# happyxtt/CNNs_SLFP_quantization

Measured on AMD Instinct MI355X. Metric: images/sec at batch 256, MobileNetV1 SLFP<3,4> ImageNet-224; % HBM roofline, higher is better.
Workload: dtype f32 (1x1 contraction: fp16 MFMA operands, f32 accumulate); 1 GPU; mobilenetv1_imagenet224: all 27 Conv2d_Q layers, SLFP<3,4> Qbits=8, NHWC, batch 256 per GPU as 2 concurrent image groups of 128 on 2 HIP streams, inputs resident in HBM; batch_per_gpu=256, global_batch=256, parallelism=batch-sharded x1, one-time RCCL broadcast of the u8 weight codes, pointwise_mfma=pw_mfma_f16x1

## Files before the change

cnns_slfp_quantization_amd/_lib.py:

```python
import ctypes
import os

_HERE = os.path.dirname(os.path.abspath(__file__))
LIB_PATH = os.path.join(_HERE, "libslfp_hip.so")

OK, ERR_BAD_ARG, ERR_SHAPE, ERR_UNSUPPORTED, ERR_ALIGNMENT, ERR_HIP = 0, -1, -2, -3, -4, -5
FMT_ACT8, FMT_W8, FMT_SFP7, FMT_EXT = 0, 1, 2, 4
LAYOUT_NCHW, LAYOUT_NHWC = 0, 1
MFMA_DEFAULT, MFMA_F16X1, MFMA_F16X3 = 0, 1, 3
OPT_SGD, OPT_DSGD, OPT_SSGD = 0, 1, 2

SYMBOLS = (
    "slfp_version", "slfp_last_error", "slfp_device_count",
    "slfp_encode_f32", "slfp_decode_f32", "slfp_quantize_f32", "slfp_quantize_layerout_f32", "slfp_absmax_f32",
    "slfp_conv2d_out_shape", "slfp_conv2d_kernel_name", "slfp_conv2d_wprep_bytes",
    "slfp_conv2d_prepare_weights", "slfp_conv2d_prepare_weights_codes", "slfp_conv2d_workspace_bytes", "slfp_conv2d_fwd", "slfp_conv2d_fwd_post",
    "slfp_linear_workspace_bytes", "slfp_linear_fwd", "slfp_linear_prepare_weights", "slfp_linear_fwd_prepared",
    "slfp_nchw_to_nhwc_f32", "slfp_nhwc_to_nchw_f32", "slfp_debug_div_mismatches",
    "slfp_debug_enc_mismatches", "slfp_enc_table_ok", "slfp_dwpw_supported", "slfp_dwpw_fwd",
    "slfp_conv2d_codes_supported", "slfp_conv2d_fwd_codes", "slfp_conv2d_fwd_codes_ws", "slfp_maxpool2d_codes", "slfp_debug_code_mismatches", "slfp_debug_reload_switches",
    "slfp_debug_enc_hl_mismatches", "slfp_sgd_step_f32",
    "slfp_conv2d_bwd_supported", "slfp_conv2d_bwd_kernel_name", "slfp_conv2d_bwd_workspace_bytes", "slfp_conv2d_bwd",
)


class ConvDesc(ctypes.Structure):
    _fields_ = [
        ("n", ctypes.c_int64), ("c_in", ctypes.c_int64), ("h", ctypes.c_int64), ("w", ctypes.c_int64),
        ("c_out", ctypes.c_int64), ("kh", ctypes.c_int64), ("kw", ctypes.c_int64),
        ("stride_h", ctypes.c_int32), ("stride_w", ctypes.c_int32), ("pad_h", ctypes.c_int32),
        ("pad_w", ctypes.c_int32), ("dil_h", ctypes.c_int32), ("dil_w", ctypes.c_int32),
        ("groups", ctypes.c_int32), ("x_layout", ctypes.c_int32), ("y_layout", ctypes.c_int32),
        ("qbits", ctypes.c_int32), ("ka", ctypes.c_float), ("kw_scale", ctypes.c_float),
        ("mfma_passes", ctypes.c_int32), ("reserved", ctypes.c_int32),
    ]


class ConvIo(ctypes.Structure):
    _fields_ = [("x_codes", ctypes.c_int32), ("y_codes", ctypes.c_int32), ("y_ka", ctypes.c_float), ("y_qbits", ctypes.c_int32)]


class SgdHparams(ctypes.Structure):
    _fields_ = [("rule", ctypes.c_int32), ("qbits", ctypes.c_int32), ("lr", ctypes.c_float), ("momentum", ctypes.c_float),
                ("damp_alpha", ctypes.c_float), ("weight_decay", ctypes.c_float), ("nesterov", ctypes.c_int32),
                ("reserved", ctypes.c_int32)]


class SlfpError(RuntimeError):
    def __init__(self, code, text):
        super().__init__(f"libslfp_hip: {text} (status {code})")
        self.code = code


_lib = None


def load():
    global _lib
    if _lib is not None:
        return _lib
    if not os.path.exists(LIB_PATH):
        raise RuntimeError(
            f"{LIB_PATH} is missing: the SLFP HIP extension is not built. "
            "Run `python -m cnns_slfp_quantization_amd.build` (needs hipcc). There is no CPU fallback.")
    import torch
    L = ctypes.CDLL(LIB_PATH)
    vp, sz, ci, cf, i64 = ctypes.c_void_p, ctypes.c_size_t, ctypes.c_int, ctypes.c_float, ctypes.c_int64
    dp = ctypes.POINTER(ConvDesc)
    sigs = {
        "slfp_version": (ci, []),
        "slfp_last_error": (ctypes.c_char_p, []),
        "slfp_device_count": (ci, []),
        "slfp_encode_f32": (ci, [vp, vp, sz, cf, ci, vp]),
        "slfp_decode_f32": (ci, [vp, vp, sz, ci, vp]),
        "slfp_quantize_f32": (ci, [vp, vp, sz, cf, ci, vp]),
        "slfp_quantize_layerout_f32": (ci, [vp, vp, sz, vp]),
        "slfp_absmax_f32": (ci, [vp, sz, vp, vp]),
        "slfp_conv2d_out_shape": (ci, [dp, ctypes.POINTER(i64), ctypes.POINTER(i64)]),
        "slfp_conv2d_kernel_name": (ctypes.c_char_p, [dp]),
        "slfp_conv2d_wprep_bytes": (sz, [dp]),
        "slfp_conv2d_prepare_weights": (ci, [dp, vp, vp, vp, vp]),
        "slfp_conv2d_prepare_weights_codes": (ci, [dp, vp, vp, vp, vp]),
        "slfp_conv2d_workspace_bytes": (sz, [dp]),
        "slfp_conv2d_fwd": (ci, [dp, vp, vp, vp, vp, vp, vp, vp]),
        "slfp_conv2d_fwd_post": (ci, [dp, vp, vp, vp, vp, vp, ci, vp, vp, vp, vp]),
        "slfp_linear_workspace_bytes": (sz, [i64, i64, i64]),
        "slfp_linear_fwd": (ci, [vp, vp, vp, vp, i64, i64, i64, cf, cf, ci, ci, vp, vp]),
        "slfp_linear_prepare_weights": (ci, [vp, vp, i64, i64, cf, ci, ci, vp]),
        "slfp_linear_fwd_prepared": (ci, [vp, vp, vp, vp, i64, i64, i64, cf, cf, ci, ci, vp]),
        "slfp_nchw_to_nhwc_f32": (ci, [vp, vp, i64, i64, i64, i64, vp]),
        "slfp_nhwc_to_nchw_f32": (ci, [vp, vp, i64, i64, i64, i64, vp]),
        "slfp_debug_div_mismatches": (ci, [cf, vp, vp]),
        "slfp_debug_enc_mismatches": (ci, [cf, ci, vp, vp]),
        "slfp_enc_table_ok": (ci, [cf, ci]),
        "slfp_dwpw_supported": (ci, [dp, dp]),
        "slfp_dwpw_fwd": (ci, [dp, dp, vp, vp, vp, vp, ci, vp, vp, vp, vp, ci, vp, vp]),
        "slfp_conv2d_codes_supported": (ci, [dp, ctypes.POINTER(ConvIo), ci, ci]),
        "slfp_conv2d_fwd_codes": (ci, [dp, ctypes.POINTER(ConvIo), vp, vp, vp, vp, vp, ci, vp, vp]),
        "slfp_conv2d_fwd_codes_ws": (ci, [dp, ctypes.POINTER(ConvIo), vp, vp, vp, vp, vp, ci, vp, vp, vp]),
        "slfp_maxpool2d_codes": (ci, [vp, vp, i64, i64, i64, i64, ci, ci, ci, ci, ci, ci, ci, vp]),
        "slfp_debug_code_mismatches": (ci, [cf, ci, vp, vp]),
        "slfp_debug_reload_switches": (None, []),
        "slfp_debug_enc_hl_mismatches": (ci, [cf, ci, vp, vp]),
        "slfp_sgd_step_f32": (ci, [ctypes.POINTER(SgdHparams), sz, vp, vp, vp, vp, vp, vp]),
        "slfp_conv2d_bwd_supported": (ci, [dp]),
        "slfp_conv2d_bwd_kernel_name": (ctypes.c_char_p, [dp]),
        "slfp_conv2d_bwd_workspace_bytes": (sz, [dp, ci, ci]),
        "slfp_conv2d_bwd": (ci, [dp, vp, vp, vp, vp, vp, vp, vp, vp]),
    }
    assert set(sigs) == set(SYMBOLS)
    for name, (res, args) in sigs.items():
        fn = getattr(L, name)
        fn.restype = res
        fn.argtypes = args
    _lib = L
    return L


def last_error():
    return load().slfp_last_error().decode("utf-8", "replace")


def check(rc):
    if rc == OK:
        return
    text = last_error()
    if rc in (ERR_BAD_ARG, ERR_SHAPE):
        raise SlfpError(rc, text)
    raise SlfpError(rc, text)
```

cnns_slfp_quantization_amd/build.py:

```python
import os
import shutil
import subprocess
import sys

HERE = os.path.dirname(os.path.abspath(__file__))
CSRC = os.path.join(HERE, "csrc")
LIB = os.path.join(HERE, "libslfp_hip.so")
SOURCES = ["codec.hip", "enc_table.hip", "conv_dw.hip", "conv_dw2.hip", "conv_dwpw.hip", "conv_dwc.hip", "conv_pw.hip", "conv_pw_codes.hip", "conv_direct.hip", "conv_dense.hip", "conv_stem_mfma.hip", "conv_stem_small.hip", "pool_codes.hip", "optim.hip", "conv_bwd.hip", "conv_abi.hip"]
FLAGS = ["--offload-arch=gfx950", "-O3", "-std=c++17", "-fPIC", "-fno-fast-math", "-ffp-contract=off",
         "-Wall", "-Wno-unused-variable", "-Wno-unused-but-set-variable"]


def _hipcc():
    for cand in (os.environ.get("HIPCC"), shutil.which("hipcc"), "/opt/rocm/bin/hipcc"):
        if cand and os.path.exists(cand):
            return cand
    raise RuntimeError("hipcc not found (set HIPCC or install ROCm)")


def needs_build():
    if not os.path.exists(LIB):
        return True
    t = os.path.getmtime(LIB)
    deps = [os.path.join(CSRC, f) for f in os.listdir(CSRC)] + [os.path.join(HERE, "..", "include", "slfp.h")]
    return any(os.path.getmtime(d) > t for d in deps)


def build(force=False, verbose=False):
    if not force and not needs_build():
        return LIB
    hipcc = _hipcc()
    extra = os.environ.get("SLFP_EXTRA_HIPCC_FLAGS", "").split()
    objdir = os.path.join(HERE, "build")
    os.makedirs(objdir, exist_ok=True)
    procs = []
    for src in SOURCES:
        obj = os.path.join(objdir, src + ".o")
        cmd = [hipcc] + FLAGS + extra + ["-c", os.path.join(CSRC, src), "-o", obj]
        if verbose:
            print(" ".join(cmd), flush=True)
        procs.append((src, obj, subprocess.Popen(cmd, stdout=subprocess.PIPE, stderr=subprocess.STDOUT, text=True)))
    objs = []
    for src, obj, p in procs:
        out, _ = p.communicate()
        if p.returncode != 0:
            raise RuntimeError(f"hipcc failed on {src}:\n{out}")
        if verbose and out.strip():
            print(out)
        objs.append(obj)
    cmd = [hipcc, "--offload-arch=gfx950", "-shared", "-fPIC", "-o", LIB] + objs
    subprocess.check_call(cmd)
    return LIB


if __name__ == "__main__":
    print(build(force="--force" in sys.argv, verbose=True))
```

cnns_slfp_quantization_amd/csrc/codec.hip:

```cpp
#include <cstdarg>
#include <mutex>
#include <map>
#include <set>
#include <utility>
#include <cstdio>
#include "slfp_device.hpp"
#include "slfp_enc.hpp"
#include "slfp_host.hpp"

namespace slfp {

static thread_local char g_err[512] = "";

void set_error(const char* fmt, ...) {
    va_list ap;
    va_start(ap, fmt);
    vsnprintf(g_err, sizeof(g_err), fmt, ap);
    va_end(ap);
}

int fail(int code, const char* fmt, ...) {
    va_list ap;
    va_start(ap, fmt);
    vsnprintf(g_err, sizeof(g_err), fmt, ap);
    va_end(ap);
    return code;
}

int check_launch(const char* what) {
    hipError_t e = hipGetLastError();
    if (e != hipSuccess) return fail(SLFP_ERR_HIP, "%s: %s", what, hipGetErrorString(e));
    return SLFP_OK;
}

const char* last_error_text() { return g_err; }

int raise_lds_limit(const void* fn, size_t lds_bytes) {
    if (lds_bytes <= 48 * 1024) return SLFP_OK;
    static std::mutex mu;
    static std::map<std::pair<int, const void*>, size_t> raised;
    int dev = 0;
    if (hipGetDevice(&dev) != hipSuccess) return check_launch("hipGetDevice");
    std::lock_guard<std::mutex> lock(mu);
    const auto key = std::make_pair(dev, fn);
    const auto it = raised.find(key);
    if (it != raised.end() && it->second >= lds_bytes) return SLFP_OK;
    if (hipFuncSetAttribute(fn, hipFuncAttributeMaxDynamicSharedMemorySize, (int)lds_bytes) != hipSuccess)
        return check_launch("hipFuncSetAttribute(MaxDynamicSharedMemorySize)");
    raised[key] = lds_bytes;
    return SLFP_OK;
}

static Switches read_switches() {
    Switches w;
    w.long_encode = std::getenv("SLFP_LONG_ENCODE") != nullptr;
    w.dw_old = std::getenv("SLFP_DW_OLD") != nullptr;
    w.pw_nostg = std::getenv("SLFP_PW_NOSTG") != nullptr;
    w.pw_notab = std::getenv("SLFP_PW_NOTAB") != nullptr;
    const char* e = std::getenv("SLFP_PW_STG_MAXKS");
    w.pw_stg_maxks = e ? atoi(e) : -1;
    e = std::getenv("SLFP_PW_NT_MIN_MB");
    w.pw_nt_min_mb = e ? atoll(e) : 0;
    e = std::getenv("SLFP_DW_NT_MIN_MB");
    w.dw_nt_min_mb = e ? atoll(e) : 30;
    w.stem_old = std::getenv("SLFP_STEM_OLD") != nullptr;
    w.pwc_slice = std::getenv("SLFP_PWC_NOSLICE") == nullptr;
    w.dense_generic = std::getenv("SLFP_DENSE_GENERIC") != nullptr;
    e = std::getenv("SLFP_DENSE_CFG");
    w.dense_cfg = e ? atoi(e) : 0;
    e = std::getenv("SLFP_DENSE_NWB");
    w.dense_nwb = e ? atoi(e) : 0;
    w.dense_res = std::getenv("SLFP_DENSE_NORES") == nullptr;
    w.dense_encx = std::getenv("SLFP_DENSE_NOENCX") == nullptr;
    w.stem_im2row = std::getenv("SLFP_STEM_IM2ROW") != nullptr;
    e = std::getenv("SLFP_PW_STREAM_MAX_KB");
    w.pw_stream_max_kb = e ? atoi(e) : 30;
    return w;
}
static Switches g_switches = read_switches();
const Switches& switches() { return g_switches; }
void reload_switches() { g_switches = read_switches(); }

int device_cu_count() {
    static std::mutex mu;
    static std::map<int, int> cus;
    int dev = 0;
    if (hipGetDevice(&dev) != hipSuccess) { (void)hipGetLastError(); return 256; }
    std::lock_guard<std::mutex> lock(mu);
    const auto it = cus.find(dev);
    if (it != cus.end()) return it->second;
    int n = 0;
    if (hipDeviceGetAttribute(&n, hipDeviceAttributeMultiprocessorCount, dev) != hipSuccess || n <= 0) { (void)hipGetLastError(); n = 256; }
    cus[dev] = n;
    return n;
}

int resident_blocks_per_cu(const void* fn, int block_threads, size_t dynamic_lds) {
    static std::mutex mu;
    static std::map<std::pair<std::pair<int, const void*>, size_t>, int> cache;
    int dev = 0;
    if (hipGetDevice(&dev) != hipSuccess) { (void)hipGetLastError(); return 1; }
    const auto key = std::make_pair(std::make_pair(dev, fn), dynamic_lds);
    std::lock_guard<std::mutex> lock(mu);
    const auto it = cache.find(key);
    if (it != cache.end()) return it->second;
    int n = 0;
    if (hipOccupancyMaxActiveBlocksPerMultiprocessor(&n, fn, block_threads, dynamic_lds) != hipSuccess || n < 1) { (void)hipGetLastError(); n = 1; }
    cache[key] = n;
    return n;
}

constexpr int kThreads = 256;

template <int FMT, int MODE>
__global__ __launch_bounds__(kThreads) void k_codec(const float* __restrict__ x, void* __restrict__ out,
                                                    size_t n, const ScaleDiv sd, int ext, int vec_ok) {
    __shared__ uint32_t sT[16];
    lut_fill<FMT>(sT);
    __syncthreads();
    const size_t nvec = vec_ok ? n / 4 : 0;
    const size_t stride = (size_t)gridDim.x * kThreads;
    for (size_t i = (size_t)blockIdx.x * kThreads + threadIdx.x; i < nvec; i += stride) {
        const float4 v = reinterpret_cast<const float4*>(x)[i];
        const uint32_t u0 = __float_as_uint(div_const(v.x, sd)), u1 = __float_as_uint(div_const(v.y, sd));
        const uint32_t u2 = __float_as_uint(div_const(v.z, sd)), u3 = __float_as_uint(div_const(v.w, sd));
        if constexpr (MODE == 0) {
            float4 r;
// ... 267 lines not shown
```

cnns_slfp_quantization_amd/csrc/conv_abi.hip:

```cpp
#include <cstring>
#include "slfp_device.hpp"
#include "slfp_codes.hpp"
#include "slfp_host.hpp"

namespace slfp {

static size_t round256(size_t b) { return (b + 255) & ~(size_t)255; }

static int make_plan_core(const slfp_conv2d_desc* d, ConvPlan* plan) {
    if (!d || !plan) return fail(SLFP_ERR_BAD_ARG, "conv2d: null descriptor");
    if (d->n <= 0 || d->c_in <= 0 || d->h <= 0 || d->w <= 0 || d->c_out <= 0 || d->kh <= 0 || d->kw <= 0)
        return fail(SLFP_ERR_SHAPE, "conv2d: non-positive size");
    if (d->stride_h <= 0 || d->stride_w <= 0 || d->dil_h <= 0 || d->dil_w <= 0 || d->pad_h < 0 || d->pad_w < 0)
        return fail(SLFP_ERR_SHAPE, "conv2d: bad stride/dilation/padding");
    if (d->groups <= 0 || d->c_in % d->groups || d->c_out % d->groups)
        return fail(SLFP_ERR_SHAPE, "conv2d: groups=%d does not divide C_in=%lld / C_out=%lld", d->groups,
                    (long long)d->c_in, (long long)d->c_out);
    if (d->qbits != 8 && d->qbits != 7)
        return fail(SLFP_ERR_BAD_ARG, "conv2d: qbits must be 8 (SLFP<3,4>) or 7 (SFP<3,3>), got %d", d->qbits);
    if ((d->x_layout != SLFP_LAYOUT_NCHW && d->x_layout != SLFP_LAYOUT_NHWC) ||
        (d->y_layout != SLFP_LAYOUT_NCHW && d->y_layout != SLFP_LAYOUT_NHWC))
        return fail(SLFP_ERR_BAD_ARG, "conv2d: unknown layout");
    if (!(d->ka > 0.f) || !(d->kw_scale > 0.f)) return fail(SLFP_ERR_BAD_ARG, "conv2d: Ka and Kw must be > 0");
    if (!scale_div_ok(d->ka) || !scale_div_ok(d->kw_scale))
// ... 172 lines not shown
    if (p.family == kPointwise || p.family == kDenseMfma || p.family == kStemMfma || p.family == kStemSmall || p.repad) {
        if (hipMemsetAsync(wprep, 0, p.wprep_bytes, stream) != hipSuccess) return check_launch("hipMemsetAsync(wprep)");
    }
    const int64_t plane = p.family == kStemMfma ? p.n_pad : p.k_pad * p.n_pad;
    const int KS = p.family == kStemMfma ? (int)p.k_pad : (int)(p.k_pad / 32);
    const unsigned grid = (unsigned)ceil_div(total, 256);
    const ScaleDiv sd = make_scale_div(d.kw_scale);
    const int ldo = p.family == kDenseMfma ? (p.passes == 3 ? 1 : 0) : (int)p.cpo;
#define SLFP_PREP(FF, CC) hipLaunchKernelGGL((k_prepare<FF, CC>), dim3(grid), dim3(256), 0, stream, w_oihw, wprep, weight_q_oihw, total, \
                                             (int)d.c_out, Cg, (int)d.kh, (int)d.kw, sd, (int)p.family, KS, plane, ldo)
    if (p.fmt_w == kFmtW8) { if (codes) SLFP_PREP(kFmtW8, true); else SLFP_PREP(kFmtW8, false); }
    else { if (codes) SLFP_PREP(kFmtSfp7, true); else SLFP_PREP(kFmtSfp7, false); }
#undef SLFP_PREP
    return check_launch("slfp weight prepare kernel");
}

static const char* family_name(const ConvPlan& p, const slfp_conv2d_desc& d) {
    if (p.family == kDirect && stem_applicable(d)) return "stem_nhwc";
    if (p.repad) {
        if (p.family == kDw3x3) return "repad+dw3x3_nhwc";
        return p.fmt_act == kFmtSfp7 ? "repad+pw_mfma_f16_exact" : (p.passes == 3 ? "repad+pw_mfma_f16x3" : "repad+pw_mfma_f16x1");
    }
    switch (p.family) {
        case kDw3x3: return "dw3x3_nhwc";
        case kPointwise: return p.fmt_act == kFmtSfp7 ? "pw_mfma_f16_exact" : (p.passes == 3 ? "pw_mfma_f16x3" : "pw_mfma_f16x1");
        case kDenseMfma: return p.fmt_act == kFmtSfp7 ? "dense_mfma_f16_exact" : (p.passes == 3 ? "dense_mfma_f16x3" : "dense_mfma_f16x1");
        case kStemMfma: return p.fmt_act == kFmtSfp7 ? "stem_mfma_f16_exact" : "stem_mfma_f16x1";
        case kStemSmall: return p.fmt_act == kFmtSfp7 ? "stem_small_mfma_f16_exact" : "stem_small_mfma_f16x1";
        default: return "direct_nhwc";
    }
}

}

using namespace slfp;

extern "C" {

int slfp_conv2d_out_shape(const slfp_conv2d_desc* d, int64_t* h_out, int64_t* w_out) {
    ConvPlan p;
    const int rc = make_plan(d, &p);
    if (rc != SLFP_OK) return rc;
    if (h_out) *h_out = p.h_out;
    if (w_out) *w_out = p.w_out;
    return SLFP_OK;
}

const char* slfp_conv2d_kernel_name(const slfp_conv2d_desc* d) {
    ConvPlan p;
    if (make_plan(d, &p) != SLFP_OK) return "invalid";
    return family_name(p, *d);
}

size_t slfp_conv2d_wprep_bytes(const slfp_conv2d_desc* d) {
    ConvPlan p;
    if (make_plan(d, &p) != SLFP_OK) return 0;
    return p.wprep_bytes;
}

int slfp_conv2d_prepare_weights(const slfp_conv2d_desc* d, const float* w_oihw, void* wprep, float* weight_q_oihw,
                                void* stream) {
    ConvPlan p;
    const int rc = make_plan(d, &p);
    if (rc != SLFP_OK) return rc;
    if (!w_oihw || !wprep) return fail(SLFP_ERR_BAD_ARG, "slfp_conv2d_prepare_weights: null pointer");
    if (!aligned16(wprep)) return fail(SLFP_ERR_ALIGNMENT, "slfp_conv2d_prepare_weights: wprep must be 16-byte aligned");
    return launch_prepare_weights(*d, p, w_oihw, wprep, weight_q_oihw, as_stream(stream));
}

int slfp_conv2d_prepare_weights_codes(const slfp_conv2d_desc* d, const uint8_t* codes_oihw, void* wprep, float* weight_q_oihw,
                                      void* stream) {
    ConvPlan p;
    const int rc = make_plan(d, &p);
    if (rc != SLFP_OK) return rc;
    if (!codes_oihw || !wprep) return fail(SLFP_ERR_BAD_ARG, "slfp_conv2d_prepare_weights_codes: null pointer");
    if (!aligned16(wprep)) return fail(SLFP_ERR_ALIGNMENT, "slfp_conv2d_prepare_weights_codes: wprep must be 16-byte aligned");
    return launch_prepare_weights(*d, p, reinterpret_cast<const float*>(codes_oihw), wprep, weight_q_oihw, as_stream(stream), true);
}

static size_t workspace_bytes_for(const slfp_conv2d_desc* d, const ConvPlan& p) {
    size_t b = 0;
    if (d->x_layout == SLFP_LAYOUT_NCHW) b += round256((size_t)d->n * d->c_in * d->h * d->w * sizeof(float));
    if (d->y_layout == SLFP_LAYOUT_NCHW) b += round256((size_t)d->n * d->c_out * p.h_out * p.w_out * sizeof(float));
    if (p.family == kDenseMfma) b += dense_mfma_workspace_bytes(*d, p.passes);
    if (p.family == kStemMfma) b += stem_mfma_workspace_bytes(*d, p.w_out);
    if (p.repad) {
        if (p.cpi != d->c_in) b += round256((size_t)d->n * d->h * d->w * p.cpi * sizeof(float));
        if (p.cpo != d->c_out) b += round256((size_t)d->n * p.h_out * p.w_out * p.cpo * sizeof(float));
        b += 3 * round256((size_t)p.cpo * sizeof(float));
    }
    return b;
}

size_t slfp_conv2d_workspace_bytes(const slfp_conv2d_desc* d) {
    ConvPlan p;
    if (make_plan(d, &p) != SLFP_OK) return 0;
    return workspace_bytes_for(d, p);
}

int slfp_conv2d_fwd(const slfp_conv2d_desc* d, const float* x, const void* wprep, const float* bias, float* y,
                    float* input_q, void* workspace, void* stream) {
    return slfp_conv2d_fwd_post(d, x, wprep, bias, nullptr, nullptr, 0, y, input_q, workspace, stream);
}

int slfp_conv2d_fwd_post(const slfp_conv2d_desc* d, const float* x, const void* wprep, const float* bias,
                         const float* post_scale, const float* post_shift, int relu, float* y, float* input_q,
// ... 221 lines not shown
```

cnns_slfp_quantization_amd/csrc/conv_dw.hip:

```cpp
#include "slfp_device.hpp"
#include "slfp_host.hpp"

namespace slfp {

constexpr int kDwThreads = 256;

struct DwParams {
    int N, H, W, C, Ho, Wo;
    int TH, TW, tiles_h, tiles_w;
    int CB, cb4_shift, cgroups;
    int pad;
    int IH, IW, IWh;
    int out_step_h, out_step_w;
    ScaleDiv sd;
    float ka, kw;
    PostOp post;
    uint32_t nblocks;
    EncArgs enc;
};

template <int V>
struct alignas(V * 4) DwVec {
    float v[V];
};
// ... 113 lines not shown
        int oh = pix0 / p.TW, ow = pix0 - oh * p.TW;
        int goh = th * p.TH + oh, gow = tw * p.TW + ow;
        float* yn = y + (size_t)n * p.Ho * p.Wo * p.C + my_c;
        int yoff = (goh * p.Wo + gow) * p.C;
        int lbase = ((oh * S) * IW + (S == 1 ? ow : 0)) * CB + my_c4 * V;
        const int y_step = (p.out_step_h * p.Wo + p.out_step_w) * p.C, y_wrap = (p.Wo - p.TW) * p.C;
        const int l_step = (p.out_step_h * S * IW + (S == 1 ? p.out_step_w : 0)) * CB;
        const int l_wrap = (S * IW - (S == 1 ? p.TW : 0)) * CB;
        const int row_pitch = IW * CB;
        for (; pix < n_pix; pix += dp) {
            if (goh < p.Ho && gow < p.Wo && c_live) {
                Vec acc = bq;
#pragma unroll
                for (int kh = 0; kh < 3; ++kh) {
                    const float* row = tile + lbase + kh * row_pitch;
#pragma unroll
                    for (int kw = 0; kw < 3; ++kw) {
                        int o;
                        if (S == 1) {
                            o = kw * CB;
                        } else {
                            const int iw = ow * 2 + kw;
                            o = ((iw & 1) * IWh + (iw >> 1)) * CB;
                        }
                        const Vec a = *reinterpret_cast<const Vec*>(row + o);
                        const Vec w = wt[kh * 3 + kw];
#pragma unroll
                        for (int e = 0; e < V; ++e) acc.v[e] = fmaf(a.v[e], w.v[e], acc.v[e]);
                    }
                }
                Vec r;
#pragma unroll
                for (int e = 0; e < V; ++e) {
                    float t = (acc.v[e] * p.ka) * p.kw;
                    if (p.post.scale) {
                        t = __builtin_fmaf(t, psc.v[e], psh.v[e]);
                        if constexpr (LO) t = layerout1(t);
                    }
                    if (p.post.relu) t = fmaxf(t, 0.f);
                    r.v[e] = t;
                }
                *reinterpret_cast<Vec*>(yn + (uint32_t)yoff) = r;
            }
            oh += p.out_step_h; goh += p.out_step_h;
            ow += p.out_step_w; gow += p.out_step_w;
            yoff += y_step; lbase += l_step;
            if (ow >= p.TW) { ow -= p.TW; gow -= p.TW; ++oh; ++goh; yoff += y_wrap; lbase += l_wrap; }
        }
    }
}

int launch_dw3x3(const slfp_conv2d_desc& d, const ConvPlan& plan, const float* x, const float* wq9c,
                 const float* bias, const PostOp& post, float* y, hipStream_t stream) {
    if (dw3x3_tile_applicable(d, plan, bias, post)) return launch_dw3x3_tile(d, plan, x, wq9c, post, y, stream);
    DwParams p;
    p.post = post;
    p.N = (int)d.n; p.H = (int)d.h; p.W = (int)d.w; p.C = (int)d.c_in;
    p.Ho = (int)plan.h_out; p.Wo = (int)plan.w_out;
    const int S = d.stride_h;
    int CB = 4;
    while (CB < 64 && p.C % (CB * 2) == 0) CB *= 2;
    if (CB < 32) {
        CB = 4;
        while (CB < 32 && CB < p.C) CB *= 2;
    }
    const int tmax = (S == 1) ? 14 : 7;
    p.TH = p.Ho < tmax ? p.Ho : tmax;
    p.TW = p.Wo < tmax ? p.Wo : tmax;
    p.tiles_h = (int)ceil_div(p.Ho, p.TH);
    p.tiles_w = (int)ceil_div(p.Wo, p.TW);
    p.IH = (p.TH - 1) * S + 3;
    p.IW = (p.TW - 1) * S + 3;
    while (CB > 4 && (size_t)p.IH * p.IW * CB * sizeof(float) > 40 * 1024) CB /= 2;
    p.CB = CB;
    p.cb4_shift = 0;
    while ((4 << p.cb4_shift) < CB) ++p.cb4_shift;
    p.cgroups = (int)ceil_div(p.C, CB);
    p.pad = d.pad_h;
    p.IWh = (p.IW + 1) / 2;
    const bool v2 = (p.C % 4) != 0;
    const int dp = kDwThreads >> (p.cb4_shift + (v2 ? 1 : 0));
    p.out_step_h = dp / p.TW; p.out_step_w = dp % p.TW;
    p.sd = make_scale_div(d.ka);
    p.ka = d.ka; p.kw = d.kw_scale;
    if ((int64_t)p.H * p.W * p.C >= (1ll << 29) || (int64_t)p.Ho * p.Wo * p.C >= (1ll << 29))
        return fail(SLFP_ERR_UNSUPPORTED, "dw3x3: one image exceeds 2^29 elements");
    const int64_t nblocks = (int64_t)p.N * p.tiles_h * p.tiles_w * p.cgroups;
    if (nblocks > 0x7FFFFFFF) return fail(SLFP_ERR_UNSUPPORTED, "dw3x3: grid too large");
    p.nblocks = (uint32_t)nblocks;
    const EncArgs* tab = act_table(d.ka, plan.fmt_act, kEncF32);
    if (tab) p.enc = *tab;
    const size_t lds = (tab ? ((kEncEntries * 8 + 15) & ~15) : 64) + (size_t)p.IH * p.IW * p.CB * sizeof(float);
    if (lds > 64 * 1024) return fail(SLFP_ERR_UNSUPPORTED, "dw3x3: tile needs %zu B of LDS", lds);
    const bool a8 = plan.fmt_act == kFmtAct8;
#define SLFP_DW_LAUNCH(FMT, SS, CBT, IWT, VV) \
    do { if (tab) hipLaunchKernelGGL((k_dw3x3<FMT, SS, CBT, IWT, VV, false, true>), dim3(p.nblocks), dim3(kDwThreads), lds, stream, x, wq9c, bias, y, p); \
         else hipLaunchKernelGGL((k_dw3x3<FMT, SS, CBT, IWT, VV>), dim3(p.nblocks), dim3(kDwThreads), lds, stream, x, wq9c, bias, y, p); } while (0)
#define SLFP_DW_LAUNCH_LO(FMT, SS, VV) \
    do { if (tab) hipLaunchKernelGGL((k_dw3x3<FMT, SS, 0, 0, VV, true, true>), dim3(p.nblocks), dim3(kDwThreads), lds, stream, x, wq9c, bias, y, p); \
         else hipLaunchKernelGGL((k_dw3x3<FMT, SS, 0, 0, VV, true>), dim3(p.nblocks), dim3(kDwThreads), lds, stream, x, wq9c, bias, y, p); } while (0)
#define SLFP_DW_BY_FMT(SS, CBT, IWT, VV) \
    do { if (a8) SLFP_DW_LAUNCH(kFmtAct8, SS, CBT, IWT, VV); else SLFP_DW_LAUNCH(kFmtSfp7, SS, CBT, IWT, VV); } while (0)
    if (p.post.layerout && p.post.scale) {
        if (a8) { if (S == 1) { if (v2) SLFP_DW_LAUNCH_LO(kFmtAct8, 1, 2); else SLFP_DW_LAUNCH_LO(kFmtAct8, 1, 4); }
                  else        { if (v2) SLFP_DW_LAUNCH_LO(kFmtAct8, 2, 2); else SLFP_DW_LAUNCH_LO(kFmtAct8, 2, 4); } }
        else    { if (S == 1) { if (v2) SLFP_DW_LAUNCH_LO(kFmtSfp7, 1, 2); else SLFP_DW_LAUNCH_LO(kFmtSfp7, 1, 4); }
// ... 20 lines not shown
```

cnns_slfp_quantization_amd/csrc/slfp_host.hpp:

```cpp
#pragma once
#include <hip/hip_runtime.h>
#include <stdint.h>
#include <stddef.h>
#include <cmath>
#include <cstring>
#include <cstdlib>
#include "../../include/slfp.h"
#include "slfp_device.hpp"
#include "slfp_enc.hpp"

namespace slfp {

void set_error(const char* fmt, ...);
int fail(int code, const char* fmt, ...);
int check_launch(const char* what);

int raise_lds_limit(const void* fn, size_t lds_bytes);

inline hipStream_t as_stream(void* s) { return reinterpret_cast<hipStream_t>(s); }
inline bool aligned16(const void* p) { return (reinterpret_cast<uintptr_t>(p) & 15u) == 0; }
inline int64_t ceil_div(int64_t a, int64_t b) { return (a + b - 1) / b; }

inline bool scale_div_ok(float d) { return std::isfinite(d) && d >= 1e-30f && d <= 1e30f; }

inline ScaleDiv make_scale_div(float d, int esh = 0) {
    ScaleDiv s;
    s.d = std::ldexp(d, -esh);
    s.r = (float)(1.0 / (double)s.d);
    return s;
}

struct Switches {
    bool long_encode, dw_old, pw_nostg, pw_notab;
    int pw_stg_maxks;
    long long pw_nt_min_mb;
    long long dw_nt_min_mb;
    bool stem_old;
    bool pwc_slice;
    bool dense_generic;
    int dense_cfg;
    int dense_nwb;
    bool dense_encx;
    bool dense_res;
    bool stem_im2row;
    int pw_stream_max_kb;
};
const Switches& switches();
void reload_switches();
inline bool long_encode_forced() { return switches().long_encode; }
inline bool dw_old_forced() { return switches().dw_old; }
inline const EncArgs* act_table(float ka, int fmt_act, int rep) {
    if (long_encode_forced()) return nullptr;
    const EncArgs* t = enc_table(ka, fmt_act, rep);
    return t->valid ? t : nullptr;
}

enum KernelFamily { kDw3x3 = 0, kPointwise = 1, kDirect = 2, kDenseMfma = 3, kStemMfma = 4, kStemSmall = 5 };

struct ConvPlan {
    KernelFamily family;
    int fmt_act;
    int fmt_w;
    int passes;
    int64_t h_out, w_out;
    float s1, s2;
    int64_t k_pad, n_pad;
    size_t wprep_bytes;
    bool repad;
    int64_t cpi, cpo;
};

int make_plan(const slfp_conv2d_desc* d, ConvPlan* plan);

int launch_quantize(const float* x, float* y, size_t n, float scale, int fmt, hipStream_t stream);
int launch_dw3x3(const slfp_conv2d_desc& d, const ConvPlan& p, const float* x, const float* wq9c,
                 const float* bias, const PostOp& post, float* y, hipStream_t stream);
bool dw3x3_tile_applicable(const slfp_conv2d_desc& d, const ConvPlan& p, const float* bias, const PostOp& post);
int launch_dw3x3_tile(const slfp_conv2d_desc& d, const ConvPlan& p, const float* x, const float* wq9c,
                      const PostOp& post, float* y, hipStream_t stream);
int launch_pointwise(const slfp_conv2d_desc& d, const ConvPlan& p, const float* x, const void* wfrag,
                     const float* bias, const PostOp& post, float* y, hipStream_t stream);
struct CodeIo {
    bool x_codes;
    bool y_codes;
    float y_ka;
    int y_fmt;
};
int resident_blocks_per_cu(const void* fn, int block_threads, size_t dynamic_lds);
int device_cu_count();
bool pwc_applicable(const slfp_conv2d_desc& d, const ConvPlan& p, int post_flags, bool y_codes);
int launch_pwc(const slfp_conv2d_desc& d, const ConvPlan& p, const uint8_t* x, const void* wfrag, const float* bias,
               const PostOp& post, void* y, bool y_codes, float y_ka, int y_fmt, hipStream_t stream);
bool stem_codes_applicable(const slfp_conv2d_desc& d, const ConvPlan& p, int post_flags);
int launch_stem_codes(const slfp_conv2d_desc& d, const ConvPlan& p, const float* x, const float* wq_hwio, const float* bias,
                      const PostOp& post, void* y, const CodeIo& io, hipStream_t stream);
bool dwc_applicable(const slfp_conv2d_desc& d, const ConvPlan& p, const float* bias, int post_flags);
int launch_dwc(const slfp_conv2d_desc& d, const ConvPlan& p, const uint8_t* x, const float* wq9c, const PostOp& post,
               void* y, bool y_codes, float y_ka, int y_fmt, hipStream_t stream);
int launch_direct(const slfp_conv2d_desc& d, const ConvPlan& p, const float* x, const float* wq_hwio,
                  const float* bias, const PostOp& post, float* y, hipStream_t stream);
bool stem_applicable(const slfp_conv2d_desc& d);
bool pointwise_stream_fits(int64_t k_pad, int64_t n_pad, int passes);
bool dense_mfma_applicable(const slfp_conv2d_desc& d, int passes);
size_t dense_mfma_workspace_bytes(const slfp_conv2d_desc& d, int passes);
int launch_dense_mfma(const slfp_conv2d_desc& d, const ConvPlan& p, const float* x, const void* wblob,
                      const float* bias, const PostOp& post, float* y, void* workspace, hipStream_t stream);
bool dense_codes_applicable(const slfp_conv2d_desc& d, const ConvPlan& p, int post_flags, bool y_codes);
int launch_dense_mfma_io(const slfp_conv2d_desc& d, const ConvPlan& p, const void* x_any, const void* wblob, const float* bias,
                         const PostOp& post, void* y_any, void* workspace, const CodeIo& io, hipStream_t stream);
int launch_prepare_weights(const slfp_conv2d_desc& d, const ConvPlan& p, const float* w_oihw, void* wprep,
                           float* weight_q_oihw, hipStream_t stream, bool codes = false);

bool stem_mfma_applicable(const slfp_conv2d_desc& d, int passes);
void stem_mfma_blob_shape(const slfp_conv2d_desc& d, int* ksub, int* nt);
size_t stem_mfma_workspace_bytes(const slfp_conv2d_desc& d, int64_t w_out);
int launch_stem_mfma(const slfp_conv2d_desc& d, const ConvPlan& p, const float* x, const void* wblob,
                     const float* bias, const PostOp& post, float* y, void* workspace, hipStream_t stream);

bool stem_small_applicable(const slfp_conv2d_desc& d, int passes);
int stem_small_tiles(const slfp_conv2d_desc& d);
int launch_stem_small(const slfp_conv2d_desc& d, const ConvPlan& p, const float* x, const void* wblob,
                      const float* bias, const PostOp& post, float* y, hipStream_t stream);
bool stem_small_codes_applicable(const slfp_conv2d_desc& d, const ConvPlan& p, int post_flags);
int launch_stem_small_io(const slfp_conv2d_desc& d, const ConvPlan& p, const float* x, const void* wblob, const float* bias,
                         const PostOp& post, void* y_any, const CodeIo& io, hipStream_t stream);

__device__ __forceinline__ uint32_t xcd_remap(uint32_t bid, uint32_t nblocks) {
    const uint32_t xcd = bid & 7u, slot = bid >> 3;
    const uint32_t q = nblocks >> 3, r = nblocks & 7u;
    const uint32_t base = xcd < r ? xcd * (q + 1u) : r * (q + 1u) + (xcd - r) * q;
    return base + slot;
}
// ... 3 lines not shown
```

include/slfp.h:

```cpp
#ifndef SLFP_H_
#define SLFP_H_

#include <stddef.h>
#include <stdint.h>

#ifdef __cplusplus
extern "C" {
#endif

#define SLFP_ABI_VERSION 1

#define SLFP_OK 0
#define SLFP_ERR_BAD_ARG (-1)
#define SLFP_ERR_SHAPE (-2)
#define SLFP_ERR_UNSUPPORTED (-3)
#define SLFP_ERR_ALIGNMENT (-4)
#define SLFP_ERR_HIP (-5)

#define SLFP_FMT_ACT8 0
#define SLFP_FMT_W8 1
#define SLFP_FMT_SFP7 2
#define SLFP_FMT_EXT 4

#define SLFP_LAYOUT_NCHW 0
#define SLFP_LAYOUT_NHWC 1

#define SLFP_MFMA_DEFAULT 0
#define SLFP_MFMA_F16X1 1
#define SLFP_MFMA_F16X3 3

int slfp_version(void);
void slfp_debug_reload_switches(void);
const char* slfp_last_error(void);
int slfp_device_count(void);


int slfp_encode_f32(const float* x, uint8_t* code, size_t n, float scale_div, int fmt, void* stream);
int slfp_decode_f32(const uint8_t* code, float* y, size_t n, int fmt, void* stream);
int slfp_quantize_f32(const float* x, float* y, size_t n, float scale_div, int fmt, void* stream);

int slfp_quantize_layerout_f32(const float* x, float* y, size_t n, void* stream);
int slfp_absmax_f32(const float* x, size_t n, float* out, void* stream);


typedef struct slfp_conv2d_desc {
    int64_t n, c_in, h, w;
    int64_t c_out, kh, kw;
    int32_t stride_h, stride_w, pad_h, pad_w, dil_h, dil_w, groups;
    int32_t x_layout, y_layout;
    int32_t qbits;
    float ka, kw_scale;
    int32_t mfma_passes;
    int32_t reserved;
} slfp_conv2d_desc;

int slfp_conv2d_out_shape(const slfp_conv2d_desc* d, int64_t* h_out, int64_t* w_out);
const char* slfp_conv2d_kernel_name(const slfp_conv2d_desc* d);

size_t slfp_conv2d_wprep_bytes(const slfp_conv2d_desc* d);
int slfp_conv2d_prepare_weights(const slfp_conv2d_desc* d, const float* w_oihw, void* wprep,
                                float* weight_q_oihw, void* stream);
int slfp_conv2d_prepare_weights_codes(const slfp_conv2d_desc* d, const uint8_t* codes_oihw, void* wprep,
                                      float* weight_q_oihw, void* stream);
size_t slfp_conv2d_workspace_bytes(const slfp_conv2d_desc* d);
int slfp_conv2d_fwd(const slfp_conv2d_desc* d, const float* x, const void* wprep, const float* bias,
                    float* y, float* input_q, void* workspace, void* stream);

#define SLFP_POST_RELU 1
#define SLFP_POST_LAYEROUT 2
int slfp_conv2d_fwd_post(const slfp_conv2d_desc* d, const float* x, const void* wprep, const float* bias,
                         const float* post_scale, const float* post_shift, int relu, float* y,
                         float* input_q, void* workspace, void* stream);

int slfp_dwpw_supported(const slfp_conv2d_desc* dw, const slfp_conv2d_desc* pw);
int slfp_dwpw_fwd(const slfp_conv2d_desc* dw, const slfp_conv2d_desc* pw, const float* x, const void* wprep_dw,
                  const float* post1_scale, const float* post1_shift, int relu1, const void* wprep_pw,
                  const float* bias_pw, const float* post2_scale, const float* post2_shift, int relu2, float* y,
                  void* stream);

typedef struct slfp_conv2d_io {
    int32_t x_codes;
    int32_t y_codes;
    float y_ka;
    int32_t y_qbits;
} slfp_conv2d_io;
int slfp_conv2d_codes_supported(const slfp_conv2d_desc* d, const slfp_conv2d_io* io, int has_bias, int relu);
int slfp_conv2d_fwd_codes(const slfp_conv2d_desc* d, const slfp_conv2d_io* io, const void* x, const void* wprep,
                          const float* bias, const float* post_scale, const float* post_shift, int relu, void* y,
                          void* stream);
int slfp_conv2d_fwd_codes_ws(const slfp_conv2d_desc* d, const slfp_conv2d_io* io, const void* x, const void* wprep,
                             const float* bias, const float* post_scale, const float* post_shift, int relu, void* y,
                             void* workspace, void* stream);
int slfp_maxpool2d_codes(const uint8_t* x, uint8_t* y, int64_t n, int64_t h, int64_t w, int64_t c, int kh, int kw, int sh, int sw,
                         int ph, int pw, int qbits, void* stream);
int slfp_debug_code_mismatches(float scale_div, int fmt, unsigned long long* out3, void* stream);

size_t slfp_linear_workspace_bytes(int64_t batch, int64_t in_f, int64_t out_f);
int slfp_linear_fwd(const float* x, const float* w, const float* bias, float* y, int64_t batch,
                    int64_t in_f, int64_t out_f, float ka, float kw_scale, int qbits, int mfma_passes,
                    void* workspace, void* stream);
int slfp_linear_prepare_weights(const float* w, void* wprep, int64_t in_f, int64_t out_f, float kw_scale,
                                int qbits, int mfma_passes, void* stream);
int slfp_linear_fwd_prepared(const float* x, const void* wprep, const float* bias, float* y, int64_t batch,
                             int64_t in_f, int64_t out_f, float ka, float kw_scale, int qbits,
                             int mfma_passes, void* stream);

int slfp_debug_div_mismatches(float scale_div, unsigned long long* out2, void* stream);

int slfp_debug_enc_mismatches(float scale_div, int fmt, unsigned long long* out2, void* stream);
int slfp_debug_enc_hl_mismatches(float scale_div, int fmt, unsigned long long* out1, void* stream);
// ... 27 lines not shown
```

Baseline: 131,500 images/sec.

## Add row-streaming depthwise 3x3 stride-2 kernel with register ring window

```diff
diff --git a/cnns_slfp_quantization_amd/_lib.py b/cnns_slfp_quantization_amd/_lib.py
--- a/cnns_slfp_quantization_amd/_lib.py
+++ b/cnns_slfp_quantization_amd/_lib.py
@@ -19,7 +19,7 @@
     "slfp_nchw_to_nhwc_f32", "slfp_nhwc_to_nchw_f32", "slfp_debug_div_mismatches",
     "slfp_debug_enc_mismatches", "slfp_enc_table_ok", "slfp_dwpw_supported", "slfp_dwpw_fwd",
     "slfp_conv2d_codes_supported", "slfp_conv2d_fwd_codes", "slfp_conv2d_fwd_codes_ws", "slfp_maxpool2d_codes", "slfp_debug_code_mismatches", "slfp_debug_reload_switches",
-    "slfp_debug_enc_hl_mismatches", "slfp_sgd_step_f32",
+    "slfp_debug_enc_hl_mismatches", "slfp_sgd_step_f32", "slfp_debug_dw3x3_variant",
     "slfp_conv2d_bwd_supported", "slfp_conv2d_bwd_kernel_name", "slfp_conv2d_bwd_workspace_bytes", "slfp_conv2d_bwd",
 )
 
@@ -78,6 +78,7 @@
         "slfp_absmax_f32": (ci, [vp, sz, vp, vp]),
         "slfp_conv2d_out_shape": (ci, [dp, ctypes.POINTER(i64), ctypes.POINTER(i64)]),
         "slfp_conv2d_kernel_name": (ctypes.c_char_p, [dp]),
+        "slfp_debug_dw3x3_variant": (ctypes.c_char_p, [dp, ci]),
         "slfp_conv2d_wprep_bytes": (sz, [dp]),
         "slfp_conv2d_prepare_weights": (ci, [dp, vp, vp, vp, vp]),
         "slfp_conv2d_prepare_weights_codes": (ci, [dp, vp, vp, vp, vp]),
diff --git a/cnns_slfp_quantization_amd/build.py b/cnns_slfp_quantization_amd/build.py
--- a/cnns_slfp_quantization_amd/build.py
+++ b/cnns_slfp_quantization_amd/build.py
@@ -6,7 +6,7 @@
 HERE = os.path.dirname(os.path.abspath(__file__))
 CSRC = os.path.join(HERE, "csrc")
 LIB = os.path.join(HERE, "libslfp_hip.so")
-SOURCES = ["codec.hip", "enc_table.hip", "conv_dw.hip", "conv_dw2.hip", "conv_dwpw.hip", "conv_dwc.hip", "conv_pw.hip", "conv_pw_codes.hip", "conv_direct.hip", "conv_dense.hip", "conv_stem_mfma.hip", "conv_stem_small.hip", "pool_codes.hip", "optim.hip", "conv_bwd.hip", "conv_abi.hip"]
+SOURCES = ["codec.hip", "enc_table.hip", "conv_dw.hip", "conv_dw2.hip", "conv_dw3.hip", "conv_dwpw.hip", "conv_dwc.hip", "conv_pw.hip", "conv_pw_codes.hip", "conv_direct.hip", "conv_dense.hip", "conv_stem_mfma.hip", "conv_stem_small.hip", "pool_codes.hip", "optim.hip", "conv_bwd.hip", "conv_abi.hip"]
 FLAGS = ["--offload-arch=gfx950", "-O3", "-std=c++17", "-fPIC", "-fno-fast-math", "-ffp-contract=off",
          "-Wall", "-Wno-unused-variable", "-Wno-unused-but-set-variable"]
 
diff --git a/cnns_slfp_quantization_amd/csrc/codec.hip b/cnns_slfp_quantization_amd/csrc/codec.hip
--- a/cnns_slfp_quantization_amd/csrc/codec.hip
+++ b/cnns_slfp_quantization_amd/csrc/codec.hip
@@ -73,6 +73,7 @@
     w.dense_res = std::getenv("SLFP_DENSE_NORES") == nullptr;
     w.dense_encx = std::getenv("SLFP_DENSE_NOENCX") == nullptr;
     w.stem_im2row = std::getenv("SLFP_STEM_IM2ROW") != nullptr;
+    w.dw_rows = parse_dw_rows(std::getenv("SLFP_DW_ROWS"));
     e = std::getenv("SLFP_PW_STREAM_MAX_KB");
     w.pw_stream_max_kb = e ? atoi(e) : 30;
     return w;
diff --git a/cnns_slfp_quantization_amd/csrc/conv_abi.hip b/cnns_slfp_quantization_amd/csrc/conv_abi.hip
--- a/cnns_slfp_quantization_amd/csrc/conv_abi.hip
+++ b/cnns_slfp_quantization_amd/csrc/conv_abi.hip
@@ -248,6 +248,15 @@
     return family_name(p, *d);
 }
 
+const char* slfp_debug_dw3x3_variant(const slfp_conv2d_desc* d, int has_post) {
+    ConvPlan p;
+    if (make_plan(d, &p) != SLFP_OK || p.family != kDw3x3) return "none";
+    static const float one = 1.f;
+    const PostOp post = {has_post ? &one : nullptr, has_post ? &one : nullptr, 0, 0};
+    if (dw3x3_rows_applicable(*d, p, nullptr, post)) return "rows";
+    return dw3x3_tile_applicable(*d, p, nullptr, post) ? "tile" : "general";
+}
+
 size_t slfp_conv2d_wprep_bytes(const slfp_conv2d_desc* d) {
     ConvPlan p;
     if (make_plan(d, &p) != SLFP_OK) return 0;
diff --git a/cnns_slfp_quantization_amd/csrc/conv_dw.hip b/cnns_slfp_quantization_amd/csrc/conv_dw.hip
--- a/cnns_slfp_quantization_amd/csrc/conv_dw.hip
+++ b/cnns_slfp_quantization_amd/csrc/conv_dw.hip
@@ -189,6 +189,7 @@
 
 int launch_dw3x3(const slfp_conv2d_desc& d, const ConvPlan& plan, const float* x, const float* wq9c,
                  const float* bias, const PostOp& post, float* y, hipStream_t stream) {
+    if (dw3x3_rows_applicable(d, plan, bias, post)) return launch_dw3x3_rows(d, plan, x, wq9c, post, y, stream);
     if (dw3x3_tile_applicable(d, plan, bias, post)) return launch_dw3x3_tile(d, plan, x, wq9c, post, y, stream);
     DwParams p;
     p.post = post;
diff --git a/cnns_slfp_quantization_amd/csrc/conv_dw3.hip b/cnns_slfp_quantization_amd/csrc/conv_dw3.hip
--- /dev/null
+++ b/cnns_slfp_quantization_amd/csrc/conv_dw3.hip
@@ -0,0 +1,194 @@
+#include "slfp_device.hpp"
+#include "slfp_enc.hpp"
+#include "slfp_host.hpp"
+
+namespace slfp {
+
+constexpr int kDwrThreads = 256;
+constexpr int kDwrWaves = kDwrThreads / 64;
+constexpr int kDwrTab = (kEncEntries * 8 + 15) & ~15;
+constexpr int kDwrTile = 7;
+
+struct DwrParams {
+    int N, H, W, C, Ho, Wo, pad;
+    int cgs;
+    int tiles_h, tiles_w;
+    uint32_t ntasks;
+    uint32_t nblocks;
+    float ka, kw;
+    int nt_out;
+    PostOp post;
+    EncArgs enc;
+};
+
+typedef float f32x4 __attribute__((ext_vector_type(4)));
+typedef unsigned int u32x4r __attribute__((ext_vector_type(4)));
+
+template <int TH, bool POST>
+__global__ __launch_bounds__(kDwrThreads, 4) void k_dw3x3_rows(const float* __restrict__ x, const float* __restrict__ wq,
+                                                               float* __restrict__ y, const DwrParams p) {
+    constexpr int S = 2, TW = kDwrTile;
+    constexpr int NR = (TH - 1) * S + 3;
+    constexpr int RING = 3 + S;
+
+    __shared__ __attribute__((aligned(16))) unsigned char smem[kDwrTab];
+    enc_fill<kDwrThreads>(reinterpret_cast<uint2*>(smem), p.enc);
+    const float r1 = p.enc.r1, lo = p.enc.lo, hi = p.enc.hi;
+
+    uint32_t t = xcd_remap(blockIdx.x, p.nblocks) * kDwrWaves + (uint32_t)__builtin_amdgcn_readfirstlane((int)(threadIdx.x >> 6));
+    const bool valid = t < p.ntasks;
+    t = valid ? t : p.ntasks - 1;
+    const int cg = (int)(t % (uint32_t)p.cgs); t /= (uint32_t)p.cgs;
+    const int tw = (int)(t % (uint32_t)p.tiles_w); t /= (uint32_t)p.tiles_w;
+    const int th = (int)(t % (uint32_t)p.tiles_h);
+    const int n = (int)(t / (uint32_t)p.tiles_h);
+    const int lane = (int)(threadIdx.x & 63), g = lane >> 3;
+    const int c = cg * 32 + (lane & 7) * 4;
+
+    f32x4 wt[9];
+#pragma unroll
+    for (int k = 0; k < 9; ++k) wt[k] = *reinterpret_cast<const f32x4*>(wq + (uint32_t)(k * p.C + c));
+    f32x4 psc = {1.f, 1.f, 1.f, 1.f}, psh = {0.f, 0.f, 0.f, 0.f};
+    if constexpr (POST) {
+        psc = *reinterpret_cast<const f32x4*>(p.post.scale + c);
+        psh = *reinterpret_cast<const f32x4*>(p.post.shift + c);
+    }
+
+    const uint32_t img_in = (uint32_t)(p.H * p.W * p.C) * 4u, img_out = (uint32_t)(p.Ho * p.Wo * p.C) * 4u;
+    const __amdgpu_buffer_rsrc_t rs = __builtin_amdgcn_make_buffer_rsrc(const_cast<float*>(x + (size_t)n * (img_in / 4u)), 0, img_in, 0x00020000);
+    const __amdgpu_buffer_rsrc_t ry = __builtin_amdgcn_make_buffer_rsrc(y + (size_t)n * (img_out / 4u), 0, img_out, 0x00020000);
+
+    const int ih0 = valid ? th * TH * S - p.pad : -0x40000000;
+    const int ow = tw * TW + g, iw0 = ow * S - p.pad;
+    const uint32_t rstep = (uint32_t)(p.W * p.C) * 4u;
+    const uint32_t rowb = (uint32_t)ih0 * rstep + (uint32_t)c * 4u;
+    uint32_t coff[2];
+    coff[0] = (unsigned)iw0 < (unsigned)p.W ? (uint32_t)(iw0 * p.C) * 4u : 0x40000000u;
+    coff[1] = (g < TW && (unsigned)(iw0 + 1) < (unsigned)p.W) ? (uint32_t)((iw0 + 1) * p.C) * 4u : 0x40000000u;
+    const int nb_addr = ((lane + 8) & 63) * 4;
+
+    f32x4 win[RING][3];
+    auto request = [&](const int j) {
+        const uint32_t roff = (unsigned)(ih0 + j) < (unsigned)p.H ? rowb + (uint32_t)j * rstep : 0x80000000u;
+#pragma unroll
+        for (int k = 0; k < 2; ++k)
+            win[j % RING][k] = __builtin_bit_cast(f32x4, __builtin_amdgcn_raw_buffer_load_b128(rs, roff + coff[k], 0, (SLFP_NT_DW & 1) ? 2 : 0));
+    };
+    auto quantize = [&](const int j0, const int nj) {
+        bool any_nan = false;
+#pragma unroll
+        for (int j = j0; j < j0 + nj; ++j)
+#pragma unroll
+            for (int k = 0; k < 2; ++k) {
+                const f32x4 v = win[j % RING][k];
+                any_nan |= enc_has_nan4(make_float4(v[0], v[1], v[2], v[3]));
+            }
+        uint32_t nan_mask = 0;
+        if (__builtin_expect(any_nan, 0)) {
+#pragma unroll
+            for (int j = j0; j < j0 + nj; ++j)
+#pragma unroll
+                for (int k = 0; k < 2; ++k) {
+                    const f32x4 v = win[j % RING][k];
+#pragma unroll
+                    for (int e = 0; e < 4; ++e)
+                        if (v[e] != v[e]) nan_mask |= 1u << (((j - j0) * 2 + k) * 4 + e);
+                }
+        }
+#pragma unroll
+        for (int j = j0; j < j0 + nj; ++j)
+#pragma unroll
+            for (int k = 0; k < 2; ++k) {
+                const f32x4 v = win[j % RING][k];
+                const float4 q = enc4_f32_raw(make_float4(v[0], v[1], v[2], v[3]), r1, lo, hi, smem);
+                win[j % RING][k] = f32x4{q.x, q.y, q.z, q.w};
+            }
+        if (__builtin_expect(nan_mask != 0, 0)) {
+#pragma unroll
+            for (int j = j0; j < j0 + nj; ++j)
+#pragma unroll
+                for (int k = 0; k < 2; ++k)
+#pragma unroll
+                    for (int e = 0; e < 4; ++e)
+                        if (nan_mask >> (((j - j0) * 2 + k) * 4 + e) & 1u) win[j % RING][k][e] = __uint_as_float(kBitsQNaN);
+        }
+#pragma unroll
+        for (int j = j0; j < j0 + nj; ++j)
+#pragma unroll
+            for (int e = 0; e < 4; ++e)
+                win[j % RING][2][e] = __int_as_float(__builtin_amdgcn_ds_bpermute(nb_addr, __float_as_int(win[j % RING][0][e])));
+    };
+
+#pragma unroll
+    for (int j = 0; j < RING && j < NR; ++j) request(j);
+
+    const int oh0 = th * TH;
+    const uint32_t ostep = (uint32_t)(p.Wo * p.C) * 4u;
+    const uint32_t ocol = (valid && g < TW && ow < p.Wo) ? (uint32_t)((oh0 * p.Wo + ow) * p.C + c) * 4u : 0x80000000u;
+
+    __syncthreads();
+
+    quantize(0, 3 - S);
+#pragma unroll
+    for (int r = 0; r < TH; ++r) {
+        quantize(r * S + 3 - S, S);
+        f32x4 acc = {0.f, 0.f, 0.f, 0.f};
+#pragma unroll
+        for (int kh = 0; kh < 3; ++kh) {
+#pragma unroll
+            for (int kw = 0; kw < 3; ++kw) {
+                const f32x4 a = win[(r * S + kh) % RING][kw];
+                const f32x4 w = wt[kh * 3 + kw];
+#pragma unroll
+                for (int e = 0; e < 4; ++e) acc[e] = fmaf(a[e], w[e], acc[e]);
+            }
+        }
+        f32x4 rr;
+#pragma unroll
+        for (int e = 0; e < 4; ++e) {
+            float u = (acc[e] * p.ka) * p.kw;
+            if constexpr (POST) u = __builtin_fmaf(u, psc[e], psh[e]);
+            if (p.post.relu) u = fmaxf(u, 0.f);
+            rr[e] = u;
+        }
+        const uint32_t so = ocol + ((oh0 + r) < p.Ho ? (uint32_t)r * ostep : 0x40000000u);
+        if (p.nt_out) __builtin_amdgcn_raw_buffer_store_b128(__builtin_bit_cast(u32x4r, rr), ry, so, 0, 2);
+        else __builtin_amdgcn_raw_buffer_store_b128(__builtin_bit_cast(u32x4r, rr), ry, so, 0, 0);
+#pragma unroll
+        for (int j = r * S + RING; j < r * S + RING + S && j < NR; ++j) request(j);
+    }
+}
+
+constexpr int kDwrRule = 0xF;
+
+bool dw3x3_rows_applicable(const slfp_conv2d_desc& d, const ConvPlan& plan, const float* bias, const PostOp& post) {
+    const int sw = switches().dw_rows;
+    if (sw == 0) return false;
+    if (!dw3x3_tile_applicable(d, plan, bias, post)) return false;
+    if (d.stride_h != 2 || d.stride_w != 2 || d.pad_h != d.pad_w) return false;
+    if ((int64_t)d.h * d.w * d.c_in * 4 > (1ll << 30) || plan.h_out * plan.w_out * d.c_in * 4 > (1ll << 30)) return false;
+    return (((sw < 0) ? kDwrRule : sw) >> dw_rows_class(plan.h_out, plan.w_out)) & 1;
+}
+
+int launch_dw3x3_rows(const slfp_conv2d_desc& d, const ConvPlan& plan, const float* x, const float* wq9c,
+                      const PostOp& post, float* y, hipStream_t stream) {
+    DwrParams p;
+    p.post = post;
+    p.N = (int)d.n; p.H = (int)d.h; p.W = (int)d.w; p.C = (int)d.c_in;
+    p.Ho = (int)plan.h_out; p.Wo = (int)plan.w_out; p.pad = d.pad_h;
+    p.cgs = p.C / 32;
+    p.tiles_h = (int)ceil_div(p.Ho, kDwrTile);
+    p.tiles_w = (int)ceil_div(p.Wo, kDwrTile);
+    const int64_t ntasks = (int64_t)p.N * p.tiles_h * p.tiles_w * p.cgs;
+    if (ntasks > 0x7FFFFFFF) return fail(SLFP_ERR_UNSUPPORTED, "dw3x3 (rows): grid too large");
+    p.ntasks = (uint32_t)ntasks;
+    p.nblocks = (uint32_t)ceil_div(ntasks, kDwrWaves);
+    p.ka = d.ka; p.kw = d.kw_scale;
+    p.nt_out = ((SLFP_NT_DW & 2) && (int64_t)p.N * p.Ho * p.Wo * p.C * 4 >= (switches().dw_nt_min_mb << 20)) ? 1 : 0;
+    p.enc = *act_table(d.ka, plan.fmt_act, kEncF32);
+    if (post.scale) hipLaunchKernelGGL((k_dw3x3_rows<kDwrTile, true>), dim3(p.nblocks), dim3(kDwrThreads), 0, stream, x, wq9c, y, p);
+    else hipLaunchKernelGGL((k_dw3x3_rows<kDwrTile, false>), dim3(p.nblocks), dim3(kDwrThreads), 0, stream, x, wq9c, y, p);
+    return check_launch("slfp dw3x3 (rows) kernel");
+}
+
+}
diff --git a/cnns_slfp_quantization_amd/csrc/slfp_host.hpp b/cnns_slfp_quantization_amd/csrc/slfp_host.hpp
--- a/cnns_slfp_quantization_amd/csrc/slfp_host.hpp
+++ b/cnns_slfp_quantization_amd/csrc/slfp_host.hpp
@@ -43,6 +43,7 @@
     bool dense_encx;
     bool dense_res;
     bool stem_im2row;
+    int dw_rows;
     int pw_stream_max_kb;
 };
 const Switches& switches();
@@ -78,6 +79,18 @@
 bool dw3x3_tile_applicable(const slfp_conv2d_desc& d, const ConvPlan& p, const float* bias, const PostOp& post);
 int launch_dw3x3_tile(const slfp_conv2d_desc& d, const ConvPlan& p, const float* x, const float* wq9c,
                       const PostOp& post, float* y, hipStream_t stream);
+bool dw3x3_rows_applicable(const slfp_conv2d_desc& d, const ConvPlan& p, const float* bias, const PostOp& post);
+int launch_dw3x3_rows(const slfp_conv2d_desc& d, const ConvPlan& p, const float* x, const float* wq9c,
+                      const PostOp& post, float* y, hipStream_t stream);
+inline int parse_dw_rows(const char* e) {
+    if (!e || !*e) return -1;
+    const long v = strtol(e, nullptr, 0);
+    return v <= 0 ? 0 : (int)(v & 0xF);
+}
+inline int dw_rows_class(int64_t h_out, int64_t w_out) {
+    const int64_t px = h_out * w_out;
+    return px >= 56 * 56 ? 0 : (px >= 28 * 28 ? 1 : (px >= 14 * 14 ? 2 : 3));
+}
 int launch_pointwise(const slfp_conv2d_desc& d, const ConvPlan& p, const float* x, const void* wfrag,
                      const float* bias, const PostOp& post, float* y, hipStream_t stream);
 struct CodeIo {
diff --git a/include/slfp.h b/include/slfp.h
--- a/include/slfp.h
+++ b/include/slfp.h
@@ -56,6 +56,7 @@
 
 int slfp_conv2d_out_shape(const slfp_conv2d_desc* d, int64_t* h_out, int64_t* w_out);
 const char* slfp_conv2d_kernel_name(const slfp_conv2d_desc* d);
+const char* slfp_debug_dw3x3_variant(const slfp_conv2d_desc* d, int has_post);
 
 size_t slfp_conv2d_wprep_bytes(const slfp_conv2d_desc* d);
 int slfp_conv2d_prepare_weights(const slfp_conv2d_desc* d, const float* w_oihw, void* wprep,
```

New measurement: 133,400 images/sec (median of 6 runs). 1.01x the previous value.
